# fatimp/SIFT3D

Measured on AMD Instinct MI355X. Metric: Mvoxel/s detect+describe (float32 volume resident in HBM), higher is better.
Workload: dtype f32; 1 GPU; 512x512x512 float32 lattice-blob volume, detect+describe, default parameters (sigma0 1.6, sigma_n 1.15, 3 levels/octave); parallelism=single GPU

## Files before the change

### include/sift3d_amd.h

```cpp
#ifndef SIFT3D_AMD_H
#define SIFT3D_AMD_H

#include <stddef.h>
#include <stdint.h>

#include "sift3d/imtypes.h"

#ifdef __cplusplus
extern "C" {
#endif

#define SIFT3D_AMD_API __attribute__((visibility("default")))


SIFT3D_AMD_API int
sift3d_amd_detect_keypoints_device(sift3d_detector *det, const float *d_volume,
                                   int nx, int ny, int nz, double ux, double uy,
                                   double uz, sift3d_keypoint_store *store);

SIFT3D_AMD_API int
sift3d_amd_image_set_units(sift3d_image *im, double ux, double uy, double uz);

SIFT3D_AMD_API int
sift3d_amd_detector_set_cuboid_extrema(sift3d_detector *det, int on);

SIFT3D_AMD_API int
sift3d_amd_detector_set_dogmax_pass(sift3d_detector *det, int on);
SIFT3D_AMD_API int
sift3d_amd_detector_set_serial_orientation(sift3d_detector *det, int on);
SIFT3D_AMD_API int
sift3d_amd_detector_set_candidate_capacity(sift3d_detector *det, int cap);
SIFT3D_AMD_API int
sift3d_amd_detector_candidate_capacity(const sift3d_detector *det);
SIFT3D_AMD_API int
sift3d_amd_detector_set_exact_descriptors(sift3d_detector *det, int mode);
SIFT3D_AMD_API int
sift3d_amd_detector_dogmax(const sift3d_detector *det, float *out, int cap);

SIFT3D_AMD_API int
sift3d_amd_image_info(const sift3d_image *im, int *dims4, double *units3);

#define SIFT3D_AMD_TIMED_BLURS 8
#define SIFT3D_AMD_NUM_TIMINGS (10 + 2 * SIFT3D_AMD_TIMED_BLURS + 4)
SIFT3D_AMD_API const double *
sift3d_amd_timings(const sift3d_detector *det);

SIFT3D_AMD_API int
sift3d_amd_build_pyramid_device(sift3d_detector *det, const float *d_volume, int nx, int ny, int nz,
                                double ux, double uy, double uz);

// ... 405 lines not shown
    float R[9];
    float cx, cy, cz;
    int32_t level;
    uint32_t row1;
    double sd;
} sift3d_hip_kp;

SIFT3D_AMD_API int
sift3d_hip_describe(const sift3d_hip_level *d_levels, const sift3d_hip_kp *d_kp,
                    uint32_t n, float *d_hist, void *stream);

SIFT3D_AMD_API size_t sift3d_hip_describe_wlut_floats(int nlevels);
SIFT3D_AMD_API int
sift3d_hip_describe_wlut(const sift3d_hip_level *d_levels, int nlevels, const sift3d_hip_kp *d_kp,
                         uint32_t n, float *d_hist, float *d_wlut, void *stream);
SIFT3D_AMD_API size_t sift3d_hip_describe_part_bytes(uint32_t n);
SIFT3D_AMD_API int
sift3d_hip_describe_parts(const sift3d_hip_level *d_levels, int nlevels, const sift3d_hip_kp *d_kp,
                          uint32_t n, uint32_t n_exact, float *d_hist, float *d_hist2, float *d_wlut,
                          void *d_part, void *stream);
SIFT3D_AMD_API int
sift3d_hip_describe_clock(const float *d_wlut, int nlevels, int exact, uint64_t *cycles, uint64_t *ticks,
                          void *stream);
SIFT3D_AMD_API int
sift3d_hip_describe_wlut2(const sift3d_hip_level *d_levels, int nlevels, const sift3d_hip_kp *d_kp,
                          uint32_t n, float *d_hist, float *d_hist2, float *d_wlut, void *stream);
SIFT3D_AMD_API int
sift3d_hip_describe_ex(const sift3d_hip_level *d_levels, int nlevels, const sift3d_hip_kp *d_kp, uint32_t n,
                       uint32_t n_exact, float *d_hist, float *d_hist2, float *d_wlut, void *stream);

SIFT3D_AMD_API int sift3d_hip_slab_count(const sift3d_hip_cand *d_cand, const int32_t *d_keep, uint32_t n,
                                         int ngl, int K, int nkey, int32_t *d_cnt, void *stream);
SIFT3D_AMD_API size_t sift3d_hip_slab_pack_scratch_bytes(uint32_t n);
SIFT3D_AMD_API int sift3d_hip_slab_pack(const sift3d_hip_level *d_levels, const sift3d_hip_cand *d_cand,
                                        const int32_t *d_keep, const float *d_R, uint32_t n, int ngl,
// ... 26 lines not shown
```

### profiles/microbench/describe_tail.py

```python
#!/usr/bin/env python3
import os
import sys, numpy as np, torch
sys.path.insert(0, os.path.dirname(os.path.dirname(os.path.dirname(os.path.abspath(__file__)))))
from sift3d_amd import api, hip
n = 512
vol = torch.empty((n, n, n), device="cuda"); hip.synth_lattice(vol, 0, 11); torch.cuda.synchronize()
det, kp, desc = api.Detector(), api.KeypointStore(), api.DescriptorStore()
assert det.detect_keypoints_device(vol.data_ptr(), n, n, n, kp) == 0
recs = kp.records()
def t(r, reps=5):
    k2 = api.KeypointStore(); k2.set_records(r)
    d2 = api.DescriptorStore()
    ts = []
    for _ in range(reps):
        assert det.extract_descriptors(k2, d2) == 0
        ts.append(det.timings()["describe"])
    return 1e3 * float(np.median(ts[1:]))
t1, t3 = t(recs), t(np.concatenate([recs] * 3))
print("whole list: %d keypoints: 1x %.3f ms, 3x %.3f ms -> per list %.3f ms, fixed part %.3f ms"
      % (len(recs), t1, t3, (t3 - t1) / 2, t1 - (t3 - t1) / 2))
for s in (0, 1, 2):
    sub = recs[recs["s"] == s]
    t1, t3 = t(sub), t(np.concatenate([sub] * 3))
    print("level s=%d: %d keypoints: 1x %.3f ms, 3x %.3f ms -> per list %.3f ms (%.2f us per keypoint and wave slot), fixed part %.3f ms"
          % (s, len(sub), t1, t3, (t3 - t1) / 2, 1e3 * (t3 - t1) / 2 * 4096 / len(sub), t1 - (t3 - t1) / 2))
```

### sift3d_amd/api.py

```python
import collections
import ctypes as C
import math
import os

import numpy as np

from . import _native

SIFT3D_SUCCESS = 0
SIFT3D_FAILURE = -1
SIFT3D_DOUBLE, SIFT3D_FLOAT, SIFT3D_INT = 0, 1, 2
TIMED_BLURS = 8
NUM_TIMINGS = 10 + 2 * TIMED_BLURS + 4

_f32p = np.ctypeslib.ndpointer(np.float32, flags="C_CONTIGUOUS")
_f64p = np.ctypeslib.ndpointer(np.float64, flags="C_CONTIGUOUS")
_i32p = np.ctypeslib.ndpointer(np.int32, flags="C_CONTIGUOUS")

_bound = None


def lib():
    global _bound
    if _bound is not None:
# ... 28 lines not shown
        "sift3d_free_descriptor_store": (None, [vp]),
        "sift3d_descriptor_store_save": (C.c_int, [C.c_char_p, vp]),
        "sift3d_descriptor_store_to_mat_rm": (C.c_int, [vp, vp]),
        "sift3d_amd_detect_keypoints_device": (C.c_int, [vp, vp, C.c_int, C.c_int, C.c_int,
                                                         C.c_double, C.c_double, C.c_double, vp]),
        "sift3d_amd_image_set_units": (C.c_int, [vp, C.c_double, C.c_double, C.c_double]),
        "sift3d_amd_timings": (C.POINTER(C.c_double), [vp]),
        "sift3d_amd_num_candidates": (C.c_int, [vp]),
        "sift3d_amd_describe_clock": (C.c_int, [vp, C.POINTER(C.c_double), C.POINTER(C.c_double)]),
        "sift3d_amd_build_pyramid_device": (C.c_int, [vp, vp, C.c_int, C.c_int, C.c_int, C.c_double, C.c_double,
                                                      C.c_double]),
        "sift3d_amd_image_info": (C.c_int, [vp, C.POINTER(C.c_int), C.POINTER(C.c_double)]),
        "sift3d_amd_detector_set_cuboid_extrema": (C.c_int, [vp, C.c_int]),
        "sift3d_amd_detector_set_dogmax_pass": (C.c_int, [vp, C.c_int]),
        "sift3d_amd_detector_set_exact_descriptors": (C.c_int, [vp, C.c_int]),
        "sift3d_amd_detector_set_serial_orientation": (C.c_int, [vp, C.c_int]),
        "sift3d_amd_detector_set_candidate_capacity": (C.c_int, [vp, C.c_int]),
        "sift3d_amd_detector_candidate_capacity": (C.c_int, [vp]),
        "sift3d_amd_detector_dogmax": (C.c_int, [vp, vp, C.c_int]),
        "sift3d_amd_copy_level": (C.c_int, [vp, C.c_int, C.c_int, C.c_int, vp, _i32p]),
        "sift3d_amd_keypoint_store_size": (C.c_int, [vp]),
        "sift3d_amd_keypoint_store_get": (C.c_int, [vp, C.c_int, C.POINTER(C.c_int),
                                                    C.POINTER(C.c_int), _f64p,
                                                    C.POINTER(C.c_float), _f32p]),
        "sift3d_amd_keypoint_store_set": (C.c_int, [vp, C.c_int, _i32p, _f64p, _f32p, _f32p]),
        "sift3d_amd_descriptor_store_size": (C.c_int, [vp]),
        "sift3d_amd_descriptor_store_set": (C.c_int, [vp, C.c_int, _f64p, _f32p, C.c_int, C.c_int, C.c_int]),
        "sift3d_amd_nn_match": (C.c_int, [vp, vp, C.c_double, _i32p]),
        "sift3d_amd_descriptor_store_keep_device": (C.c_int, [vp, C.c_int]),
        "sift3d_amd_descriptor_store_xyz_all": (C.c_int, [vp, _f64p]),
# ... 253 lines not shown
    def set_sigma_n(self, v):
        return lib().sift3d_detector_set_sigma_n(self.h, float(v))

    def set_sigma0(self, v):
        return lib().sift3d_detector_set_sigma0(self.h, float(v))

    def set_cuboid_extrema(self, on):
        return lib().sift3d_amd_detector_set_cuboid_extrema(self.h, int(bool(on)))

    def set_serial_orientation(self, on):
        return lib().sift3d_amd_detector_set_serial_orientation(self.h, int(bool(on)))

    def set_exact_descriptors(self, mode):
        return lib().sift3d_amd_detector_set_exact_descriptors(self.h, int(mode))

    def set_dogmax_pass(self, on):
        return lib().sift3d_amd_detector_set_dogmax_pass(self.h, int(bool(on)))

    def set_candidate_capacity(self, cap):
        if lib().sift3d_amd_detector_set_candidate_capacity(self.h, int(cap)) != 0:
            raise ValueError("sift3d_amd_detector_set_candidate_capacity(%r)" % (cap,))

    def candidate_capacity(self):
        return lib().sift3d_amd_detector_candidate_capacity(self.h)

    def dogmax(self):
        out = np.zeros(1024, np.float32)
        n = lib().sift3d_amd_detector_dogmax(self.h, out.ctypes.data, out.size)
        if n < 0:
            raise RuntimeError("sift3d_amd_detector_dogmax")
# ... 619 lines not shown
```

### sift3d_amd/csrc/sift3d_describe.hip

```cpp
#include "sift3d_kernels_common.h"
#include "sift3d_math.h"

#include <algorithm>
#include <cmath>
#include <cstdlib>

struct FaceRec {
    float v0[3], e1[3], e2[3], t[3], q[3], e2q, idx[3];
};
static_assert(sizeof(FaceRec) == SIFT3D_HIP_FACE_FLOATS * 4, "face record layout");

__constant__ float c_face16[20 * 16];
__constant__ int c_bin_off[12];
__constant__ int c_oct_face[32];

constexpr int DQ = 256;
constexpr int HIST_USED = 800;
constexpr int HIST_LDS = 800;
constexpr int FACE_STRIDE = 20;
constexpr int RROW = 36;

#ifdef SIFT3D_AMD_DIAG
#define DESC_ABLATE_ARG , int ablate
#define DESC_ABLATE(bit) (ablate & (bit))
// ... 74 lines not shown
        const float sq = (float)k * u2;
        const float arg = -0.5f * sq / sig2;
        tab[WL_HEAD + k] = arg >= -150.0f ? s3d_expf(arg) : 0.0f;
    }
}

constexpr int DWAVES = 4;
constexpr int DPARTS = 4;

template <bool EXACT>
__global__ __launch_bounds__(64 * DWAVES) void k_describe(const sift3d_hip_level *__restrict__ levels,
                                                 const sift3d_hip_kp *__restrict__ kps, uint32_t first,
                                                 uint32_t n,
                                                 float *__restrict__ out, float *__restrict__ out2,
                                                 const float *__restrict__ wlut,
                                                 uint32_t *__restrict__ work, float *__restrict__ part,
                                                 uint32_t *__restrict__ done DESC_ABLATE_ARG)
{
    __shared__ float hist_[DWAVES][2 * HIST_LDS];
    __shared__ __attribute__((aligned(16))) float rec_[DWAVES][14][RROW];
    __shared__ int queue_[DWAVES][DQ];
    __shared__ __attribute__((aligned(16))) float sface[20 * FACE_STRIDE];
    __shared__ int soct[32];
    __shared__ uint64_t sexp[32];
    const int wv = __builtin_amdgcn_readfirstlane((int)(threadIdx.x >> 6));
    const int lane = threadIdx.x & 63;
    float *const hist = hist_[wv];
    float(*const mw)[RROW] = &rec_[wv][0];
    float(*const bw)[RROW] = &rec_[wv][8];
    int(*const ab)[RROW] = reinterpret_cast<int(*)[RROW]>(&rec_[wv][11]);
    int *const queue = queue_[wv];
    for (int i = threadIdx.x; i < 20 * 16; i += 64 * DWAVES)
        sface[(i >> 4) * FACE_STRIDE + (i & 15)] = c_face16[i];
    if (threadIdx.x < 32) {
        soct[threadIdx.x] = c_oct_face[threadIdx.x];
        sexp[threadIdx.x] = s3d_exp2_tab[threadIdx.x];
    }
    __syncthreads();
    const bool probe = work && blockIdx.x == 0 && threadIdx.x == 0;
    long long probe_c0 = 0, probe_w0 = 0;
    if (probe) {
        probe_c0 = clock64();
        probe_w0 = wall_clock64();
    }
    const bool split = !EXACT && part != nullptr;
    for (bool first_pass = true;; first_pass = false) {
    uint32_t item;
    if (work) {
        uint32_t t = 0;
        if (lane == 0)
            t = atomicAdd(work, 1u);
        item = (uint32_t)__builtin_amdgcn_readfirstlane((int)t);
    } else {
        if (!first_pass)
            break;
        item = blockIdx.x * DWAVES + wv;
    }
    const uint32_t ki = first + (split ? item / DPARTS : item);
    const int pp = split ? (int)(item % DPARTS) : 0;
    if (ki >= n)
        break;
    for (int i = lane; i < 2 * HIST_LDS; i += 64)
        hist[i] = 0.0f;
    wave_sync();
    const sift3d_hip_kp K = kps[ki];
    const sift3d_hip_level L = levels[K.level];
    const uint32_t orow = K.row1 ? K.row1 - 1 : ki;
    const float *__restrict__ wtab = nullptr;
    const int icx = (int)K.cx, icy = (int)K.cy, icz = (int)K.cz;
    if (wlut) {
        const float *tab = wlut + (size_t)K.level * WL_STRIDE;
        const long long sdbits = ((long long)__float_as_int(tab[3]) << 32) | (unsigned)__float_as_int(tab[2]);
        if (tab[0] == 1.0f && sdbits == __double_as_longlong(K.sd) && (float)icx == K.cx &&
            (float)icy == K.cy && (float)icz == K.cz)
// ... 410 lines not shown
    }
#ifdef SIFT3D_AMD_DIAG
    if (lane == 0)
        atomicAdd(&g_desc_voxels, (unsigned long long)diag_voxels);
#endif
    commit_tail(0);
    commit_tail(1);
    wave_sync();
    const float trunc = 0.2f * 128.0f / 768.0f;
    if (!EXACT) {
        for (int i = lane; i < HIST_USED; i += 64)
            hist[i] = hist[i] + hist[HIST_LDS + i];
        wave_sync();
    }
    if (split) {
        float *mine = part + ((size_t)(ki - first) * DPARTS + (size_t)pp) * HIST_USED;
        for (int i = lane; i < HIST_USED; i += 64)
            __hip_atomic_store(mine + i, hist[i], __ATOMIC_RELAXED, __HIP_MEMORY_SCOPE_AGENT);
        asm volatile("s_waitcnt vmcnt(0)" ::: "memory");
        uint32_t arrived = 0;
        if (lane == 0)
            arrived = __hip_atomic_fetch_add(done + (ki - first), 1u, __ATOMIC_RELAXED, __HIP_MEMORY_SCOPE_AGENT);
        arrived = (uint32_t)__builtin_amdgcn_readfirstlane((int)arrived);
        if (arrived != DPARTS - 1) {
            wave_sync();
            continue;
        }
        const float *all = part + (size_t)(ki - first) * DPARTS * HIST_USED;
        for (int i = lane; i < HIST_USED; i += 64) {
            float v = __hip_atomic_load(all + i, __ATOMIC_RELAXED, __HIP_MEMORY_SCOPE_AGENT);
#pragma unroll
            for (int q = 1; q < DPARTS; q++)
                v = v + __hip_atomic_load(all + (size_t)q * HIST_USED + i, __ATOMIC_RELAXED, __HIP_MEMORY_SCOPE_AGENT);
            hist[i] = v;
        }
        wave_sync();
    }
    for (int pass = 0; pass < 2; pass++) {
        double norm = 0.0;
        if (EXACT) {
            for (int c = 0; c < 64; c++)
#pragma unroll
                for (int b = 0; b < 12; b++) {
// ... 556 lines not shown
__attribute__((visibility("default"))) unsigned long long sift3d_amd_diag_desc_voxels(void)
{
    unsigned long long v = 0, z = 0;
    (void)hipDeviceSynchronize();
    (void)hipMemcpyFromSymbol(&v, HIP_SYMBOL(g_desc_voxels), sizeof(v));
    (void)hipMemcpyToSymbol(HIP_SYMBOL(g_desc_voxels), &z, sizeof(z));
    return v;
}
#endif

size_t sift3d_hip_describe_wlut_floats(int nlevels)
{
    return nlevels > 0 ? (size_t)nlevels * WL_STRIDE + WL_COUNTERS : 0;
}

static unsigned describe_grid(uint32_t count, bool counted)
{
    const unsigned need = (count + DWAVES - 1) / DWAVES;
    if (!counted)
        return need;
    static int cus = 0;
    if (!cus) {
        int dev = 0;
        hipDeviceProp_t prop;
        if (hipGetDevice(&dev) == hipSuccess && hipGetDeviceProperties(&prop, dev) == hipSuccess)
            cus = prop.multiProcessorCount;
        if (cus < 1)
            cus = 256;
    }
    const unsigned cap = (unsigned)cus * 4u;
    return need < cap ? need : cap;
}

size_t sift3d_hip_describe_part_bytes(uint32_t n)
{
    return n ? (size_t)n * DPARTS * HIST_USED * sizeof(float) + (size_t)n * sizeof(uint32_t) : 0;
}

static int describe_launch(const sift3d_hip_level *d_levels, int nlevels, const sift3d_hip_kp *d_kp, uint32_t n,
                           uint32_t n_exact, float *d_hist, float *d_hist2, const float *d_wlut,
                           void *d_part, void *stream)
{
    if (n_exact > n)
        n_exact = n;
#ifdef SIFT3D_AMD_DIAG
    static int ablate = getenv("SIFT3D_AMD_DESC_ABLATE") ? atoi(getenv("SIFT3D_AMD_DESC_ABLATE")) : 0;
#define DESC_ABLATE_PASS , ablate
#else
#define DESC_ABLATE_PASS
#endif
    uint32_t *work = d_wlut ? reinterpret_cast<uint32_t *>(const_cast<float *>(d_wlut) + (size_t)nlevels * WL_STRIDE)
                            : nullptr;
    if (n_exact) {
        hipLaunchKernelGGL(k_describe<true>, dim3(describe_grid(n_exact, work != nullptr)), dim3(64 * DWAVES), 0,
                           (hipStream_t)stream, d_levels, d_kp, 0u, n_exact, d_hist, d_hist2, d_wlut,
                           work, (float *)nullptr, (uint32_t *)nullptr DESC_ABLATE_PASS);
        LAUNCH_CHECK();
    }
    if (n > n_exact) {
        const uint32_t nf = n - n_exact;
        void *tmp = nullptr;
        if (!d_part) {
            HIPCHK(hipMalloc(&tmp, sift3d_hip_describe_part_bytes(nf)));
            d_part = tmp;
        }
        float *parts = reinterpret_cast<float *>(d_part);
        uint32_t *done = reinterpret_cast<uint32_t *>(parts + (size_t)nf * DPARTS * HIST_USED);
        hipError_t e = hipMemsetAsync(done, 0, (size_t)nf * sizeof(uint32_t), (hipStream_t)stream);
        if (e == hipSuccess) {
            hipLaunchKernelGGL(k_describe<false>, dim3(describe_grid(nf * DPARTS, work != nullptr)),
                               dim3(64 * DWAVES), 0, (hipStream_t)stream, d_levels, d_kp, n_exact, n, d_hist,
                               d_hist2, d_wlut, work ? work + 1 : nullptr, parts, done DESC_ABLATE_PASS);
            e = hipGetLastError();
        }
        if (tmp) {
            const hipError_t e2 = hipStreamSynchronize((hipStream_t)stream);
            (void)hipFree(tmp);
            if (e == hipSuccess)
                e = e2;
        }
        if (e != hipSuccess)
            return fail("k_describe", e, __FILE__, __LINE__);
    }
#undef DESC_ABLATE_PASS
    return SIFT3D_SUCCESS;
}

int sift3d_hip_describe(const sift3d_hip_level *d_levels, const sift3d_hip_kp *d_kp, uint32_t n,
                        float *d_hist, void *stream)
{
    if (!n)
        return SIFT3D_SUCCESS;
    return describe_launch(d_levels, 0, d_kp, n, 0, d_hist, nullptr, nullptr, nullptr, stream);
}

int sift3d_hip_describe_parts(const sift3d_hip_level *d_levels, int nlevels, const sift3d_hip_kp *d_kp,
                              uint32_t n, uint32_t n_exact, float *d_hist, float *d_hist2, float *d_wlut,
                              void *d_part, void *stream)
{
    if (!n)
        return SIFT3D_SUCCESS;
    if (!d_wlut || nlevels < 1)
        return describe_launch(d_levels, 0, d_kp, n, n_exact, d_hist, d_hist2, nullptr, d_part, stream);
    hipLaunchKernelGGL(k_desc_wlut, dim3(nlevels), dim3(256), 0, (hipStream_t)stream, d_levels, nlevels,
                       d_wlut);
    return describe_launch(d_levels, nlevels, d_kp, n, n_exact, d_hist, d_hist2, d_wlut, d_part, stream);
}

int sift3d_hip_describe_ex(const sift3d_hip_level *d_levels, int nlevels, const sift3d_hip_kp *d_kp,
                           uint32_t n, uint32_t n_exact, float *d_hist, float *d_hist2, float *d_wlut,
                           void *stream)
{
    return sift3d_hip_describe_parts(d_levels, nlevels, d_kp, n, n_exact, d_hist, d_hist2, d_wlut, nullptr,
                                     stream);
}

int sift3d_hip_describe_clock(const float *d_wlut, int nlevels, int exact, uint64_t *cycles, uint64_t *ticks,
                              void *stream)
{
    if (!d_wlut || nlevels < 1 || !cycles || !ticks)
        return SIFT3D_FAILURE;
// ... 146 lines not shown
```

### sift3d_amd/csrc/sift3d_host.c

```c
#include <float.h>
#include <math.h>
#include <stdint.h>
#include <stdio.h>
#include <stdlib.h>
#include <string.h>
#include <time.h>
#include <zlib.h>
#include <omp.h>
#include <dlfcn.h>
#include <pthread.h>

#include "../../include/sift3d/imutil.h"
#include "../../include/sift3d/sift.h"
#include "../../include/sift3d_amd.h"

#define ERR(...) fprintf(stderr, __VA_ARGS__)

#define NFACES 20
#define NVERT 12
#define DESC_NUMEL 768
#define SLAB_LEN 500

static const double peak_thresh_default = 0.1;
static const int num_kp_levels_default = 3;
// ... 1017 lines not shown

int sift3d_amd_detector_set_serial_orientation(sift3d_detector *d, int on)
{
    if (!d)
        return SIFT3D_FAILURE;
    d->orient_serial = on != 0;
    return SIFT3D_SUCCESS;
}

int sift3d_amd_detector_set_exact_descriptors(sift3d_detector *d, int mode)
{
    if (!d || mode < -1 || mode > 1)
        return SIFT3D_FAILURE;
    d->exact_desc = mode;
    return SIFT3D_SUCCESS;
}

static int pack_bits(long v)
{
    int b = 0;
    for (; v > 0; v >>= 1)
        b++;
    return b;
}

static int exact_desc_keypoint(int mode, double sd, int o, const double *units)
{
    double side;
    if (mode)
        return mode > 0;
// ... 1084 lines not shown
        sift3d_hip_free(desc->d_hist);
        desc->d_cap = 0;
        desc->d_hist = (float *)sift3d_hip_malloc(sizeof(float) * DESC_NUMEL * desc->cap);
        if (!desc->d_hist)
            return SIFT3D_FAILURE;
        desc->d_cap = desc->cap;
    }
    d->t_pending &= ~2;
    rng = range_start("sift3d: descriptors");
    sift3d_hip_event_record(d->ev[6], d->stream);
    {
        float *dev_view = (float *)sift3d_hip_host_device_ptr(desc->hist);
        const sift3d_hip_kp *kp_view = (const sift3d_hip_kp *)sift3d_hip_host_device_ptr(d->h_kp);
        const size_t need = sift3d_hip_describe_part_bytes((uint32_t)(num - (int)n_exact));
        if (need > d->dpart_bytes) {
            sift3d_hip_free(d->d_dpart);
            d->dpart_bytes = 0;
            d->d_dpart = sift3d_hip_malloc(need + need / 8);
            if (!d->d_dpart)
                return SIFT3D_FAILURE;
            d->dpart_bytes = need + need / 8;
        }
        if (!dev_view || !kp_view ||
            sift3d_hip_describe_parts(d->d_levels, d->num_octaves * d->ngl, kp_view, (uint32_t)num,
                                      (uint32_t)n_exact, dev_view, desc->keep_device ? desc->d_hist : NULL,
                                      d->d_wlut, need ? d->d_dpart : NULL, d->stream))
            return SIFT3D_FAILURE;
    }
    sift3d_hip_event_record(d->ev[7], d->stream);
    for (i = 0; i < num; i++) {
        const keypoint_t *k = kp->buf + i;
        const double f = ldexp(1.0, k->o);
        desc->xyzsd[4 * (size_t)i] = k->xd * f;
        desc->xyzsd[4 * (size_t)i + 1] = k->yd * f;
        desc->xyzsd[4 * (size_t)i + 2] = k->zd * f;
        desc->xyzsd[4 * (size_t)i + 3] = k->sd;
// ... 74 lines not shown
```

### sift3d_amd/csrc/sift3d_sharded.c

```c

#include <dlfcn.h>

#define SH_MAX_K 8
#define SH_MAX_NGL (SH_MAX_K + 3)
#define SH_MAX_NDL (SH_MAX_K + 2)
#define SH_MAX_OCT 32
#define SH_MAX_WORLD 64

typedef struct {
    float *t;
    int off, nloc;
    int z0, z1;
    int nz_glob;
} sh_level;

typedef struct {
    int32_t o, s, x, y, z;
    float R[9];
} sh_gkp;

struct sift3d_amd_sharded {
    sift3d_amd_transport T;
    int rank, world;
    double peak_thresh, corner_thresh, sigma_n, sigma0;
// ... 919 lines not shown
    S->t[0] = 1e-3 * sift3d_hip_event_elapsed_ms(S->ev0, S->ev1);
    S->t[3] = 1e-3 * sift3d_hip_event_elapsed_ms(S->ev1, S->ev2);
    S->t[4] = 1e-3 * sift3d_hip_event_elapsed_ms(S->ev2, S->ev3);
    S->t[5] = now_s() - S->t_gather0;
    S->t[6] = 1e-3 * sift3d_hip_event_elapsed_ms(S->ev4, S->ev0);
    S->t[1] = now_s() - t_start;
    return SIFT3D_SUCCESS;
}

int sift3d_amd_sharded_describe(sift3d_amd_sharded *S, const sift3d_keypoint_store *kp,
                                sift3d_descriptor_store *desc, int *own_idx, int *n_own)
{
    const double t_start = now_s();
    int n = 0, num;
    size_t n_exact = 0;
    if (!S || !kp || !desc || !own_idx || !n_own)
        return SIFT3D_FAILURE;
    num = (int)kp->num;
    {
        const int nt = host_threads((size_t)num);
        size_t pre[HOST_THREADS_MAX + 1], total = 0;
        int bad = 0;
        pre[0] = 0;
#pragma omp parallel num_threads(nt) reduction(| : bad)
        {
            const int nth = omp_get_num_threads(), t = omp_get_thread_num();
            const size_t lo = (size_t)num * t / nth, hi = (size_t)num * (t + 1) / nth;
            size_t q, jj = 0;
#define SH_OWN(k_) (S->world == 1 || ((k_)->zd >= (double)S->bounds[(k_)->o][S->rank] &&          \
                                      (k_)->zd < (double)S->bounds[(k_)->o][S->rank + 1]))
// ... 51 lines not shown
        const uint32_t cap = (uint32_t)n + (uint32_t)n / 4 + 256;
        sift3d_hip_host_free(S->h_kp);
        S->kp_cap = 0;
        S->h_kp = (sift3d_hip_kp *)sift3d_hip_host_alloc(sizeof(sift3d_hip_kp) * (size_t)cap);
        if (!S->h_kp)
            return SIFT3D_FAILURE;
        S->kp_cap = cap;
    }
    {
        enum { LVM = 16 };
        const int nt = host_threads((size_t)n);
        const int s_exact = exact_desc_first_level(S->exact_desc, S->ngl, S->K, S->sigma0, S->units) - 1;
        size_t cnt[HOST_THREADS_MAX][LVM], start[HOST_THREADS_MAX][LVM];
        if (S->K > LVM)
            return SIFT3D_FAILURE;
        memset(cnt, 0, sizeof(cnt));
#pragma omp parallel num_threads(nt)
        {
            const int nth = omp_get_num_threads(), t = omp_get_thread_num();
            const size_t lo = (size_t)n * t / nth, hi = (size_t)n * (t + 1) / nth;
            size_t q;
            for (q = lo; q < hi; q++)
                cnt[t][kp->buf[own_idx[q]].s]++;
#pragma omp barrier
#pragma omp single
            {
                size_t p = 0;
                int lv, u;
                for (lv = S->K - 1; lv >= 0; lv--) {
                    if (lv == s_exact - 1)
// ... 13 lines not shown
                memcpy(r->R, k->R, sizeof(r->R));
                r->cx = (float)k->xd; r->cy = (float)k->yd; r->cz = (float)k->zd;
                r->level = k->o * S->ngl + k->s + 1;
                r->row1 = (uint32_t)q + 1u;
                r->sd = k->sd;
                desc->xyzsd[4 * q] = k->xd * f;
                desc->xyzsd[4 * q + 1] = k->yd * f;
                desc->xyzsd[4 * q + 2] = k->zd * f;
                desc->xyzsd[4 * q + 3] = k->sd;
            }
        }
    }
    {
        float *dev_view = (float *)sift3d_hip_host_device_ptr(desc->hist);
        const sift3d_hip_kp *kp_view = (const sift3d_hip_kp *)sift3d_hip_host_device_ptr(S->h_kp);
        const size_t need = sift3d_hip_describe_part_bytes((uint32_t)n - (uint32_t)n_exact);
        if (need > S->dpart_bytes) {
            sift3d_hip_free(S->d_dpart);
            S->dpart_bytes = 0;
            S->d_dpart = sift3d_hip_malloc(need + need / 8);
            if (!S->d_dpart)
                return SIFT3D_FAILURE;
            S->dpart_bytes = need + need / 8;
        }
        if (!dev_view || !kp_view ||
            sift3d_hip_describe_parts(S->d_levels, S->num_octaves * S->ngl, kp_view, (uint32_t)n,
                                      (uint32_t)n_exact, dev_view, NULL, S->d_wlut, need ? S->d_dpart : NULL,
                                      S->stream) ||
            sift3d_hip_stream_sync(S->stream))
            return SIFT3D_FAILURE;
    }
    S->t[2] = now_s() - t_start;
    return SIFT3D_SUCCESS;
}

int sift3d_amd_sharded_gather_descriptors(sift3d_amd_sharded *S, const sift3d_keypoint_store *kp,
                                          const sift3d_descriptor_store *own, const int *own_idx, int n_own,
                                          sift3d_descriptor_store *all, int root)
{
    const int W = S ? S->world : 0;
    size_t num, maxn = 0, blk, q;
    size_t cnt[SH_MAX_WORLD];
    uint32_t *map = NULL;
// ... 244 lines not shown
```

### sift3d_amd/hip.py

```python
import ctypes as C

import numpy as np

from . import _native

MAX_TAPS = 65
FACE_FLOATS = 19


class FirArgs(C.Structure):
    _fields_ = [("src", C.c_void_p), ("dst", C.c_void_p), ("nx", C.c_int), ("ny", C.c_int),
                ("nz", C.c_int), ("axis", C.c_int), ("width", C.c_int),
                ("taps", C.POINTER(C.c_float)), ("unit_factor", C.c_float), ("n_glob", C.c_int),
                ("off", C.c_int), ("z_lo", C.c_int), ("z_hi", C.c_int), ("variant", C.c_int)]


class ExtremaLevel(C.Structure):
    _fields_ = [("prev", C.c_void_p), ("cur", C.c_void_p), ("next", C.c_void_p),
                ("d_absmax", C.c_void_p), ("z_lo", C.c_int), ("z_hi", C.c_int), ("tag", C.c_int)]


class Level(C.Structure):
    _fields_ = [("data", C.c_void_p), ("nx", C.c_int), ("ny", C.c_int), ("nz", C.c_int),
                ("z_off", C.c_int), ("nz_glob", C.c_int), ("ux", C.c_float), ("uy", C.c_float),
# ... 51 lines not shown
        "sift3d_hip_subtract_absmax": (C.c_int, [vp, vp, vp, C.c_size_t, vp, vp]),
        "sift3d_hip_dog_stack": (C.c_int, [C.POINTER(vp), C.POINTER(vp), C.c_int, C.c_size_t, vp, vp]),
        "sift3d_hip_host_device_ptr": (vp, [vp]),
        "sift3d_hip_downsample2": (C.c_int, [vp, C.c_int, C.c_int, vp, C.c_int, C.c_int, C.c_int, vp]),
        "sift3d_hip_extrema_work_bytes": (C.c_size_t, [C.c_int, C.c_int, C.c_int, C.c_int]),
        "sift3d_hip_extrema": (C.c_int, [C.POINTER(ExtremaLevel), C.c_int, C.c_int, C.c_int, C.c_int,
                                         C.c_double, vp, C.c_uint32, vp, vp, C.c_size_t, vp]),
        "sift3d_hip_extrema_mode": (C.c_int, [C.POINTER(ExtremaLevel), C.c_int, C.c_int, C.c_int, C.c_int,
                                              C.c_double, C.c_int, vp, C.c_uint32, vp, vp, C.c_size_t, vp]),
        "sift3d_hip_orient": (C.c_int, [vp, vp, C.c_uint32, C.c_double, vp, vp, vp]),
        "sift3d_hip_orient_tab_bytes": (C.c_size_t, [C.c_int, C.c_uint32]),
        "sift3d_hip_orient_tab": (C.c_int, [vp, C.c_int, vp, C.c_uint32, C.c_double, vp, vp, vp, C.c_uint32, vp]),
        "sift3d_hip_orient_tab_part": (C.c_int, [vp, C.c_int, C.c_int, C.c_int, vp, C.c_uint32, C.c_uint32,
                                                 C.c_double, vp, vp, vp, C.c_uint32, C.c_int, vp]),
        "sift3d_hip_describe": (C.c_int, [vp, vp, C.c_uint32, vp, vp]),
        "sift3d_hip_set_mesh": (C.c_int, [C.POINTER(C.c_float)]),
        "sift3d_hip_synth_lattice": (C.c_int, [vp, C.c_int, C.c_int, C.c_int, C.c_int, C.c_uint64, vp]),
        "sift3d_hip_warp_affine": (C.c_int, [vp, C.c_int, C.c_int, C.c_int, vp, C.c_int, C.c_int, C.c_int,
                                             C.POINTER(C.c_double), C.c_int, C.c_float, vp]),
        "sift3d_hip_warp_tps": (C.c_int, [vp, C.c_int, C.c_int, C.c_int, vp, C.c_int, C.c_int, C.c_int,
                                          C.POINTER(C.c_double), vp, C.c_int, C.c_int, C.c_float, vp]),
        "sift3d_hip_warp_tps_launches": (C.c_int, [C.c_int, C.c_int, C.c_int, C.c_int]),
        "sift3d_hip_affine_field": (C.c_int, [vp, C.c_int, C.c_int, C.c_int, C.POINTER(C.c_double), vp]),
        "sift3d_hip_tps_field": (C.c_int, [vp, C.c_int, C.c_int, C.c_int, C.POINTER(C.c_double), vp, C.c_int, vp]),
        "sift3d_hip_tps_field_launches": (C.c_int, [C.c_int, C.c_int, C.c_int, C.c_int]),
        "sift3d_hip_warp_field": (C.c_int, [vp, C.c_int, C.c_int, C.c_int, C.c_int, vp, C.c_int, C.c_int, C.c_int,
                                            vp, C.c_int, C.c_float, vp]),
        "sift3d_hip_jacobian_det": (C.c_int, [vp, C.c_int, C.c_int, C.c_int, vp, vp, vp]),
        "sift3d_hip_bspline_work_floats": (C.c_size_t, [C.c_int, C.c_int, C.c_int]),
        "sift3d_hip_bspline_prefilter": (C.c_int, [vp, C.c_int, C.c_int, C.c_int, C.c_int, vp, vp, vp]),
# ... 697 lines not shown
    if parts is None:
        _check(L.sift3d_hip_orient_tab(d_levels.data_ptr(), nlevels, dc.data_ptr(), n, float(corner_thresh),
                                       R.data_ptr(), keep.data_ptr(), tab.data_ptr(), n, current_stream()),
               "sift3d_hip_orient_tab")
    else:
        streams = [torch.cuda.Stream(), torch.cuda.Stream()]
        for slot, (lv_lo, lv_hi, first, m) in enumerate(parts):
            _check(L.sift3d_hip_orient_tab_part(d_levels.data_ptr(), nlevels, lv_lo, lv_hi, dc.data_ptr(), first, m,
                                                float(corner_thresh), R.data_ptr(), keep.data_ptr(),
                                                tab.data_ptr(), n, slot, streams[slot].cuda_stream),
                   "sift3d_hip_orient_tab_part")
    torch.cuda.synchronize()
    return R.cpu().numpy(), keep.cpu().numpy()


def describe(d_levels, kps):
    import torch
    n = len(kps)
    if n == 0:
        return np.zeros((0, 768), np.float32)
    dk = torch.from_numpy(np.ascontiguousarray(kps).view(np.uint8)).cuda()
    hist = torch.empty((n, 768), dtype=torch.float32, device="cuda")
    _check(lib().sift3d_hip_describe(d_levels.data_ptr(), dk.data_ptr(), n, hist.data_ptr(),
                                     current_stream()), "sift3d_hip_describe")
    return hist.cpu().numpy()
```

Before: 3960 Mvoxel/s.

## Split only the tail of describe windows into parts, run the rest whole

Before this, every fast-path descriptor window was split into DPARTS partial histograms, and those partials were merged through global scratch and atomic counters. Now the first windows run whole in one wave. Only the last tail, sized to about half a grid of waves from the CU count, is split to balance the end of the launch. This cuts scratch traffic, atomics and the memset for most keypoints, and shrinks scratch allocation; the fallback malloc becomes stream-ordered (hipMallocAsync/hipFreeAsync) instead of a synchronize-then-free. The sharded path has to compute a per-shard tail count consistent with the global ordering, which adds host-side bookkeeping.

```diff
diff --git a/include/sift3d_amd.h b/include/sift3d_amd.h
--- a/include/sift3d_amd.h
+++ b/include/sift3d_amd.h
@@ -34,6 +34,8 @@
 sift3d_amd_detector_candidate_capacity(const sift3d_detector *det);
 SIFT3D_AMD_API int
 sift3d_amd_detector_set_exact_descriptors(sift3d_detector *det, int mode);
+SIFT3D_AMD_API size_t
+sift3d_amd_detector_describe_scratch_bytes(const sift3d_detector *det);
 SIFT3D_AMD_API int
 sift3d_amd_detector_dogmax(const sift3d_detector *det, float *out, int cap);
 
@@ -469,11 +471,18 @@
 SIFT3D_AMD_API int
 sift3d_hip_describe_wlut(const sift3d_hip_level *d_levels, int nlevels, const sift3d_hip_kp *d_kp,
                          uint32_t n, float *d_hist, float *d_wlut, void *stream);
+SIFT3D_AMD_API uint32_t sift3d_hip_describe_tail(uint32_t n_fast);
 SIFT3D_AMD_API size_t sift3d_hip_describe_part_bytes(uint32_t n);
+SIFT3D_AMD_API size_t sift3d_hip_describe_part_cap(void);
 SIFT3D_AMD_API int
 sift3d_hip_describe_parts(const sift3d_hip_level *d_levels, int nlevels, const sift3d_hip_kp *d_kp,
                           uint32_t n, uint32_t n_exact, float *d_hist, float *d_hist2, float *d_wlut,
                           void *d_part, void *stream);
+SIFT3D_AMD_API int
+sift3d_hip_describe_parts_tail(const sift3d_hip_level *d_levels, int nlevels, const sift3d_hip_kp *d_kp,
+                               uint32_t n, uint32_t n_exact, float *d_hist, float *d_hist2, float *d_wlut,
+                               void *d_part, uint32_t n_tail, void *stream);
+SIFT3D_AMD_API void sift3d_hip_describe_set_tail(long long t);
 SIFT3D_AMD_API int
 sift3d_hip_describe_clock(const float *d_wlut, int nlevels, int exact, uint64_t *cycles, uint64_t *ticks,
                           void *stream);
diff --git a/profiles/microbench/describe_tail.py b/profiles/microbench/describe_tail.py
--- a/profiles/microbench/describe_tail.py
+++ b/profiles/microbench/describe_tail.py
@@ -16,9 +16,15 @@
         assert det.extract_descriptors(k2, d2) == 0
         ts.append(det.timings()["describe"])
     return 1e3 * float(np.median(ts[1:]))
-t1, t3 = t(recs), t(np.concatenate([recs] * 3))
-print("whole list: %d keypoints: 1x %.3f ms, 3x %.3f ms -> per list %.3f ms, fixed part %.3f ms"
-      % (len(recs), t1, t3, (t3 - t1) / 2, t1 - (t3 - t1) / 2))
+grid = 2 * hip.describe_tail(1 << 30)
+for name, T in (("whole windows", 0), ("1/2 grid", grid // 2), ("1 grid", grid), ("2 grids", 2 * grid),
+                ("every window", 1 << 30)):
+    hip.describe_set_tail(T)
+    t1, t2, t3 = t(recs), t(np.concatenate([recs] * 2)), t(np.concatenate([recs] * 3))
+    print("T = %s (%d): %d keypoints: 1x %.3f ms, 2x %.3f ms, 3x %.3f ms -> per list %.3f ms, fixed part %.3f ms, "
+          "scratch %.1f MB" % (name, hip.describe_tail(1 << 30), len(recs), t1, t2, t3, (t3 - t1) / 2,
+                               t1 - (t3 - t1) / 2, det.describe_scratch_bytes() / 1e6), flush=True)
+hip.describe_set_tail(None)
 for s in (0, 1, 2):
     sub = recs[recs["s"] == s]
     t1, t3 = t(sub), t(np.concatenate([sub] * 3))
diff --git a/sift3d_amd/api.py b/sift3d_amd/api.py
--- a/sift3d_amd/api.py
+++ b/sift3d_amd/api.py
@@ -66,6 +66,7 @@
         "sift3d_amd_detector_set_cuboid_extrema": (C.c_int, [vp, C.c_int]),
         "sift3d_amd_detector_set_dogmax_pass": (C.c_int, [vp, C.c_int]),
         "sift3d_amd_detector_set_exact_descriptors": (C.c_int, [vp, C.c_int]),
+        "sift3d_amd_detector_describe_scratch_bytes": (C.c_size_t, [vp]),
         "sift3d_amd_detector_set_serial_orientation": (C.c_int, [vp, C.c_int]),
         "sift3d_amd_detector_set_candidate_capacity": (C.c_int, [vp, C.c_int]),
         "sift3d_amd_detector_candidate_capacity": (C.c_int, [vp]),
@@ -349,6 +350,9 @@
     def set_exact_descriptors(self, mode):
         return lib().sift3d_amd_detector_set_exact_descriptors(self.h, int(mode))
 
+    def describe_scratch_bytes(self):
+        return int(lib().sift3d_amd_detector_describe_scratch_bytes(self.h))
+
     def set_dogmax_pass(self, on):
         return lib().sift3d_amd_detector_set_dogmax_pass(self.h, int(bool(on)))
 
diff --git a/sift3d_amd/csrc/sift3d_describe.hip b/sift3d_amd/csrc/sift3d_describe.hip
--- a/sift3d_amd/csrc/sift3d_describe.hip
+++ b/sift3d_amd/csrc/sift3d_describe.hip
@@ -112,7 +112,8 @@
                                                  uint32_t n,
                                                  float *__restrict__ out, float *__restrict__ out2,
                                                  const float *__restrict__ wlut,
-                                                 uint32_t *__restrict__ work, float *__restrict__ part,
+                                                 uint32_t *__restrict__ work, uint32_t nwhole,
+                                                 float *__restrict__ part,
                                                  uint32_t *__restrict__ done DESC_ABLATE_ARG)
 {
     __shared__ float hist_[DWAVES][2 * HIST_LDS];
@@ -141,7 +142,6 @@
         probe_c0 = clock64();
         probe_w0 = wall_clock64();
     }
-    const bool split = !EXACT && part != nullptr;
     for (bool first_pass = true;; first_pass = false) {
     uint32_t item;
     if (work) {
@@ -154,8 +154,10 @@
             break;
         item = blockIdx.x * DWAVES + wv;
     }
-    const uint32_t ki = first + (split ? item / DPARTS : item);
-    const int pp = split ? (int)(item % DPARTS) : 0;
+    const bool split = !EXACT && item >= nwhole;
+    const uint32_t srow = split ? (item - nwhole) / DPARTS : 0u;
+    const uint32_t ki = first + (split ? nwhole + srow : item);
+    const int pp = split ? (int)((item - nwhole) % DPARTS) : 0;
     if (ki >= n)
         break;
     for (int i = lane; i < 2 * HIST_LDS; i += 64)
@@ -596,19 +598,22 @@
         wave_sync();
     }
     if (split) {
-        float *mine = part + ((size_t)(ki - first) * DPARTS + (size_t)pp) * HIST_USED;
+#if defined(__HIP_DEVICE_COMPILE__) && !(defined(__gfx942__) || defined(__gfx950__))
+#error "k_describe: the hand-over of split windows is validated on gfx942 / gfx950 only (stores counted by vmcnt)"
+#endif
+        float *mine = part + ((size_t)srow * DPARTS + (size_t)pp) * HIST_USED;
         for (int i = lane; i < HIST_USED; i += 64)
             __hip_atomic_store(mine + i, hist[i], __ATOMIC_RELAXED, __HIP_MEMORY_SCOPE_AGENT);
         asm volatile("s_waitcnt vmcnt(0)" ::: "memory");
         uint32_t arrived = 0;
         if (lane == 0)
-            arrived = __hip_atomic_fetch_add(done + (ki - first), 1u, __ATOMIC_RELAXED, __HIP_MEMORY_SCOPE_AGENT);
+            arrived = __hip_atomic_fetch_add(done + srow, 1u, __ATOMIC_RELAXED, __HIP_MEMORY_SCOPE_AGENT);
         arrived = (uint32_t)__builtin_amdgcn_readfirstlane((int)arrived);
         if (arrived != DPARTS - 1) {
             wave_sync();
             continue;
         }
-        const float *all = part + (size_t)(ki - first) * DPARTS * HIST_USED;
+        const float *all = part + (size_t)srow * DPARTS * HIST_USED;
         for (int i = lane; i < HIST_USED; i += 64) {
             float v = __hip_atomic_load(all + i, __ATOMIC_RELAXED, __HIP_MEMORY_SCOPE_AGENT);
 #pragma unroll
@@ -1195,11 +1200,8 @@
     return nlevels > 0 ? (size_t)nlevels * WL_STRIDE + WL_COUNTERS : 0;
 }
 
-static unsigned describe_grid(uint32_t count, bool counted)
-{
-    const unsigned need = (count + DWAVES - 1) / DWAVES;
-    if (!counted)
-        return need;
+static unsigned describe_cus()
+{
     static int cus = 0;
     if (!cus) {
         int dev = 0;
@@ -1209,18 +1211,53 @@
         if (cus < 1)
             cus = 256;
     }
-    const unsigned cap = (unsigned)cus * 4u;
+    return (unsigned)cus;
+}
+
+static unsigned describe_grid(uint32_t count, bool counted)
+{
+    const unsigned need = (count + DWAVES - 1) / DWAVES;
+    if (!counted)
+        return need;
+    const unsigned cap = describe_cus() * 4u;
     return need < cap ? need : cap;
 }
 
+constexpr unsigned DTAIL_GRIDS_X2 = 1;
+static long long g_tail_override = -1;
+
+uint32_t sift3d_hip_describe_tail(uint32_t n_fast)
+{
+    const unsigned long long t = g_tail_override >= 0
+                                     ? (unsigned long long)g_tail_override
+                                     : (unsigned long long)describe_cus() * 4u * DWAVES * DTAIL_GRIDS_X2 / 2u;
+    return n_fast < t ? n_fast : (uint32_t)t;
+}
+
+void sift3d_hip_describe_set_tail(long long t)
+{
+    g_tail_override = t < 0 ? -1 : (t > 0xffffffffll ? 0xffffffffll : t);
+}
+
+static size_t describe_rows_bytes(uint32_t rows)
+{
+    return rows ? (size_t)rows * DPARTS * HIST_USED * sizeof(float) + (size_t)rows * sizeof(uint32_t) : 0;
+}
+
 size_t sift3d_hip_describe_part_bytes(uint32_t n)
 {
-    return n ? (size_t)n * DPARTS * HIST_USED * sizeof(float) + (size_t)n * sizeof(uint32_t) : 0;
-}
-
+    return describe_rows_bytes(sift3d_hip_describe_tail(n));
+}
+
+size_t sift3d_hip_describe_part_cap(void)
+{
+    return describe_rows_bytes(describe_cus() * 4u * DWAVES * DTAIL_GRIDS_X2 / 2u);
+}
+
+constexpr uint32_t DESC_TAIL_RULE = 0xffffffffu;
 static int describe_launch(const sift3d_hip_level *d_levels, int nlevels, const sift3d_hip_kp *d_kp, uint32_t n,
                            uint32_t n_exact, float *d_hist, float *d_hist2, const float *d_wlut,
-                           void *d_part, void *stream)
+                           void *d_part, uint32_t n_tail, void *stream)
 {
     if (n_exact > n)
         n_exact = n;
@@ -1235,28 +1272,36 @@
     if (n_exact) {
         hipLaunchKernelGGL(k_describe<true>, dim3(describe_grid(n_exact, work != nullptr)), dim3(64 * DWAVES), 0,
                            (hipStream_t)stream, d_levels, d_kp, 0u, n_exact, d_hist, d_hist2, d_wlut,
-                           work, (float *)nullptr, (uint32_t *)nullptr DESC_ABLATE_PASS);
+                           work, n_exact, (float *)nullptr, (uint32_t *)nullptr DESC_ABLATE_PASS);
         LAUNCH_CHECK();
     }
     if (n > n_exact) {
         const uint32_t nf = n - n_exact;
+        if (n_tail == DESC_TAIL_RULE)
+            n_tail = sift3d_hip_describe_tail(nf);
+        if (n_tail > nf)
+            n_tail = nf;
+        const uint32_t nwhole = nf - n_tail;
+        if ((unsigned long long)nwhole + (unsigned long long)DPARTS * n_tail > 0xfffffff0ull)
+            return fail("k_describe", hipErrorInvalidValue, __FILE__, __LINE__);
         void *tmp = nullptr;
-        if (!d_part) {
-            HIPCHK(hipMalloc(&tmp, sift3d_hip_describe_part_bytes(nf)));
+        hipError_t e = hipSuccess;
+        if (n_tail && !d_part) {
+            HIPCHK(hipMallocAsync(&tmp, describe_rows_bytes(n_tail), (hipStream_t)stream));
             d_part = tmp;
         }
         float *parts = reinterpret_cast<float *>(d_part);
-        uint32_t *done = reinterpret_cast<uint32_t *>(parts + (size_t)nf * DPARTS * HIST_USED);
-        hipError_t e = hipMemsetAsync(done, 0, (size_t)nf * sizeof(uint32_t), (hipStream_t)stream);
+        uint32_t *done = n_tail ? reinterpret_cast<uint32_t *>(parts + (size_t)n_tail * DPARTS * HIST_USED) : nullptr;
+        if (n_tail)
+            e = hipMemsetAsync(done, 0, (size_t)n_tail * sizeof(uint32_t), (hipStream_t)stream);
         if (e == hipSuccess) {
-            hipLaunchKernelGGL(k_describe<false>, dim3(describe_grid(nf * DPARTS, work != nullptr)),
+            hipLaunchKernelGGL(k_describe<false>, dim3(describe_grid(nwhole + n_tail * DPARTS, work != nullptr)),
                                dim3(64 * DWAVES), 0, (hipStream_t)stream, d_levels, d_kp, n_exact, n, d_hist,
-                               d_hist2, d_wlut, work ? work + 1 : nullptr, parts, done DESC_ABLATE_PASS);
+                               d_hist2, d_wlut, work ? work + 1 : nullptr, nwhole, parts, done DESC_ABLATE_PASS);
             e = hipGetLastError();
         }
         if (tmp) {
-            const hipError_t e2 = hipStreamSynchronize((hipStream_t)stream);
-            (void)hipFree(tmp);
+            const hipError_t e2 = hipFreeAsync(tmp, (hipStream_t)stream);
             if (e == hipSuccess)
                 e = e2;
         }
@@ -1272,20 +1317,28 @@
 {
     if (!n)
         return SIFT3D_SUCCESS;
-    return describe_launch(d_levels, 0, d_kp, n, 0, d_hist, nullptr, nullptr, nullptr, stream);
+    return describe_launch(d_levels, 0, d_kp, n, 0, d_hist, nullptr, nullptr, nullptr, DESC_TAIL_RULE, stream);
+}
+
+int sift3d_hip_describe_parts_tail(const sift3d_hip_level *d_levels, int nlevels, const sift3d_hip_kp *d_kp,
+                                   uint32_t n, uint32_t n_exact, float *d_hist, float *d_hist2, float *d_wlut,
+                                   void *d_part, uint32_t n_tail, void *stream)
+{
+    if (!n)
+        return SIFT3D_SUCCESS;
+    if (!d_wlut || nlevels < 1)
+        return describe_launch(d_levels, 0, d_kp, n, n_exact, d_hist, d_hist2, nullptr, d_part, n_tail, stream);
+    hipLaunchKernelGGL(k_desc_wlut, dim3(nlevels), dim3(256), 0, (hipStream_t)stream, d_levels, nlevels,
+                       d_wlut);
+    return describe_launch(d_levels, nlevels, d_kp, n, n_exact, d_hist, d_hist2, d_wlut, d_part, n_tail, stream);
 }
 
 int sift3d_hip_describe_parts(const sift3d_hip_level *d_levels, int nlevels, const sift3d_hip_kp *d_kp,
                               uint32_t n, uint32_t n_exact, float *d_hist, float *d_hist2, float *d_wlut,
                               void *d_part, void *stream)
 {
-    if (!n)
-        return SIFT3D_SUCCESS;
-    if (!d_wlut || nlevels < 1)
-        return describe_launch(d_levels, 0, d_kp, n, n_exact, d_hist, d_hist2, nullptr, d_part, stream);
-    hipLaunchKernelGGL(k_desc_wlut, dim3(nlevels), dim3(256), 0, (hipStream_t)stream, d_levels, nlevels,
-                       d_wlut);
-    return describe_launch(d_levels, nlevels, d_kp, n, n_exact, d_hist, d_hist2, d_wlut, d_part, stream);
+    return sift3d_hip_describe_parts_tail(d_levels, nlevels, d_kp, n, n_exact, d_hist, d_hist2, d_wlut, d_part,
+                                          DESC_TAIL_RULE, stream);
 }
 
 int sift3d_hip_describe_ex(const sift3d_hip_level *d_levels, int nlevels, const sift3d_hip_kp *d_kp,
diff --git a/sift3d_amd/csrc/sift3d_host.c b/sift3d_amd/csrc/sift3d_host.c
--- a/sift3d_amd/csrc/sift3d_host.c
+++ b/sift3d_amd/csrc/sift3d_host.c
@@ -1055,6 +1055,11 @@
         return SIFT3D_FAILURE;
     d->exact_desc = mode;
     return SIFT3D_SUCCESS;
+}
+
+size_t sift3d_amd_detector_describe_scratch_bytes(const sift3d_detector *d)
+{
+    return d ? d->dpart_bytes : 0;
 }
 
 static int pack_bits(long v)
@@ -2169,12 +2174,13 @@
         const sift3d_hip_kp *kp_view = (const sift3d_hip_kp *)sift3d_hip_host_device_ptr(d->h_kp);
         const size_t need = sift3d_hip_describe_part_bytes((uint32_t)(num - (int)n_exact));
         if (need > d->dpart_bytes) {
+            const size_t cap = sift3d_hip_describe_part_cap(), want = need > cap ? need : cap;
             sift3d_hip_free(d->d_dpart);
             d->dpart_bytes = 0;
-            d->d_dpart = sift3d_hip_malloc(need + need / 8);
+            d->d_dpart = sift3d_hip_malloc(want);
             if (!d->d_dpart)
                 return SIFT3D_FAILURE;
-            d->dpart_bytes = need + need / 8;
+            d->dpart_bytes = want;
         }
         if (!dev_view || !kp_view ||
             sift3d_hip_describe_parts(d->d_levels, d->num_octaves * d->ngl, kp_view, (uint32_t)num,
diff --git a/sift3d_amd/csrc/sift3d_sharded.c b/sift3d_amd/csrc/sift3d_sharded.c
--- a/sift3d_amd/csrc/sift3d_sharded.c
+++ b/sift3d_amd/csrc/sift3d_sharded.c
@@ -957,6 +957,7 @@
     const double t_start = now_s();
     int n = 0, num;
     size_t n_exact = 0;
+    int s_first_exact = 0;
     if (!S || !kp || !desc || !own_idx || !n_own)
         return SIFT3D_FAILURE;
     num = (int)kp->num;
@@ -1038,6 +1039,7 @@
         size_t cnt[HOST_THREADS_MAX][LVM], start[HOST_THREADS_MAX][LVM];
         if (S->K > LVM)
             return SIFT3D_FAILURE;
+        s_first_exact = s_exact;
         memset(cnt, 0, sizeof(cnt));
 #pragma omp parallel num_threads(nt)
         {
@@ -1081,19 +1083,49 @@
     {
         float *dev_view = (float *)sift3d_hip_host_device_ptr(desc->hist);
         const sift3d_hip_kp *kp_view = (const sift3d_hip_kp *)sift3d_hip_host_device_ptr(S->h_kp);
-        const size_t need = sift3d_hip_describe_part_bytes((uint32_t)n - (uint32_t)n_exact);
+        size_t gcnt[16] = { 0 }, g_fast = 0, skip, q, q_t = 0;
+        uint32_t g_tail, n_tail = 0;
+        int lv, lv_t = -1;
+        const int lv_fast = s_first_exact <= 0 ? 0 : s_first_exact < S->K ? s_first_exact : S->K;
+        size_t need;
+        for (q = 0; q < kp->num; q++)
+            gcnt[kp->buf[q].s]++;
+        for (lv = 0; lv < lv_fast; lv++)
+            g_fast += gcnt[lv];
+        g_tail = sift3d_hip_describe_tail((uint32_t)g_fast);
+        skip = g_fast - g_tail;
+        for (lv = lv_fast - 1; lv >= 0; lv--) {
+            if (skip < gcnt[lv]) {
+                lv_t = lv;
+                break;
+            }
+            skip -= gcnt[lv];
+        }
+        if (lv_t >= 0 && skip) {
+            size_t seen = 0;
+            for (q = 0; q < kp->num; q++)
+                if (kp->buf[q].s == lv_t && seen++ == skip)
+                    break;
+            q_t = q;
+        }
+        for (q = 0; q < (size_t)n && lv_t >= 0; q++) {
+            const keypoint_t *k = kp->buf + own_idx[q];
+            n_tail += k->s < lv_t || (k->s == lv_t && (size_t)own_idx[q] >= q_t);
+        }
+        need = sift3d_hip_describe_part_bytes(g_tail);
         if (need > S->dpart_bytes) {
+            const size_t cap = sift3d_hip_describe_part_cap(), want = need > cap ? need : cap;
             sift3d_hip_free(S->d_dpart);
             S->dpart_bytes = 0;
-            S->d_dpart = sift3d_hip_malloc(need + need / 8);
+            S->d_dpart = sift3d_hip_malloc(want);
             if (!S->d_dpart)
                 return SIFT3D_FAILURE;
-            S->dpart_bytes = need + need / 8;
+            S->dpart_bytes = want;
         }
         if (!dev_view || !kp_view ||
-            sift3d_hip_describe_parts(S->d_levels, S->num_octaves * S->ngl, kp_view, (uint32_t)n,
-                                      (uint32_t)n_exact, dev_view, NULL, S->d_wlut, need ? S->d_dpart : NULL,
-                                      S->stream) ||
+            sift3d_hip_describe_parts_tail(S->d_levels, S->num_octaves * S->ngl, kp_view, (uint32_t)n,
+                                           (uint32_t)n_exact, dev_view, NULL, S->d_wlut,
+                                           n_tail ? S->d_dpart : NULL, n_tail, S->stream) ||
             sift3d_hip_stream_sync(S->stream))
             return SIFT3D_FAILURE;
     }
diff --git a/sift3d_amd/hip.py b/sift3d_amd/hip.py
--- a/sift3d_amd/hip.py
+++ b/sift3d_amd/hip.py
@@ -89,6 +89,12 @@
         "sift3d_hip_orient_tab_part": (C.c_int, [vp, C.c_int, C.c_int, C.c_int, vp, C.c_uint32, C.c_uint32,
                                                  C.c_double, vp, vp, vp, C.c_uint32, C.c_int, vp]),
         "sift3d_hip_describe": (C.c_int, [vp, vp, C.c_uint32, vp, vp]),
+        "sift3d_hip_describe_wlut_floats": (C.c_size_t, [C.c_int]),
+        "sift3d_hip_describe_tail": (C.c_uint32, [C.c_uint32]),
+        "sift3d_hip_describe_set_tail": (None, [C.c_longlong]),
+        "sift3d_hip_describe_part_bytes": (C.c_size_t, [C.c_uint32]),
+        "sift3d_hip_describe_part_cap": (C.c_size_t, []),
+        "sift3d_hip_describe_parts": (C.c_int, [vp, C.c_int, vp, C.c_uint32, C.c_uint32, vp, vp, vp, vp, vp]),
         "sift3d_hip_set_mesh": (C.c_int, [C.POINTER(C.c_float)]),
         "sift3d_hip_synth_lattice": (C.c_int, [vp, C.c_int, C.c_int, C.c_int, C.c_int, C.c_uint64, vp]),
         "sift3d_hip_warp_affine": (C.c_int, [vp, C.c_int, C.c_int, C.c_int, vp, C.c_int, C.c_int, C.c_int,
@@ -816,13 +822,42 @@
     return R.cpu().numpy(), keep.cpu().numpy()
 
 
-def describe(d_levels, kps):
-    import torch
+def describe(d_levels, kps, stream=None):
+    import torch
+    n = len(kps)
+    if n == 0:
+        _check(lib().sift3d_hip_describe(d_levels.data_ptr(), None, 0, None,
+                                         current_stream() if stream is None else stream), "sift3d_hip_describe")
+        return np.zeros((0, 768), np.float32)
+    dk = torch.from_numpy(np.ascontiguousarray(kps).view(np.uint8)).cuda()
+    hist = torch.empty((n, 768), dtype=torch.float32, device="cuda")
+    _check(lib().sift3d_hip_describe(d_levels.data_ptr(), dk.data_ptr(), n, hist.data_ptr(),
+                                     current_stream() if stream is None else stream), "sift3d_hip_describe")
+    torch.cuda.synchronize()
+    return hist.cpu().numpy()
+
+
+def describe_set_tail(t):
+    lib().sift3d_hip_describe_set_tail(-1 if t is None else int(t))
+
+
+def describe_tail(n_fast):
+    return int(lib().sift3d_hip_describe_tail(int(n_fast)))
+
+
+def describe_parts(d_levels, nlevels, kps, n_exact=0, scratch=True):
+    import torch
+    L = lib()
     n = len(kps)
     if n == 0:
         return np.zeros((0, 768), np.float32)
     dk = torch.from_numpy(np.ascontiguousarray(kps).view(np.uint8)).cuda()
     hist = torch.empty((n, 768), dtype=torch.float32, device="cuda")
-    _check(lib().sift3d_hip_describe(d_levels.data_ptr(), dk.data_ptr(), n, hist.data_ptr(),
-                                     current_stream()), "sift3d_hip_describe")
+    wlut = torch.empty(L.sift3d_hip_describe_wlut_floats(nlevels), dtype=torch.float32, device="cuda")
+    nb = L.sift3d_hip_describe_part_bytes(n - min(n, n_exact)) if scratch else 0
+    part = torch.empty(max(nb, 1), dtype=torch.uint8, device="cuda")
+    _check(L.sift3d_hip_describe_parts(d_levels.data_ptr(), nlevels, dk.data_ptr(), n, n_exact, hist.data_ptr(),
+                                       None, wlut.data_ptr(), part.data_ptr() if nb else None,
+                                       current_stream()), "sift3d_hip_describe_parts")
+    torch.cuda.synchronize()
     return hist.cpu().numpy()
```

Measured after the change: 3960 Mvoxel/s, median of 2. Within noise of the previous version (+0.0%).
